# smoggy-P/gym-Drone2D-ActivePerception

Hardware: NVIDIA B200
Metric: env-steps/sec (higher is better)
Workload: dtype f64

## Files before the change

### gym_drone2d_activeperception_b200/csrc/d2d_step.cuh

```cuda
#pragma once
#include "d2d_state.cuh"
#include "d2d_math.cuh"

#if defined(D2D_COLD_NOINLINE) && D2D_COLD_NOINLINE
#define D2D_COLD __noinline__
#else
#define D2D_COLD __forceinline__
#endif

__device__ __forceinline__ uint32_t d2d_smem_u32(const void *p) { return (uint32_t)__cvta_generic_to_shared(p); }
__device__ __forceinline__ void d2d_mbar_init(uint64_t *bar, uint32_t count) {
    asm volatile("mbarrier.init.shared::cta.b64 [%0], %1;" ::"r"(d2d_smem_u32(bar)), "r"(count) : "memory");
    asm volatile("fence.mbarrier_init.release.cluster;" ::: "memory");
}
__device__ __forceinline__ void d2d_mbar_expect_tx(uint64_t *bar, uint32_t bytes) {
    asm volatile("mbarrier.arrive.expect_tx.shared::cta.b64 _, [%0], %1;" ::"r"(d2d_smem_u32(bar)), "r"(bytes) : "memory");
}
__device__ __forceinline__ void d2d_bulk_g2s(void *dst_smem, const void *src_gmem, uint32_t bytes, uint64_t *bar) {
    asm volatile("cp.async.bulk.shared::cluster.global.mbarrier::complete_tx::bytes [%0], [%1], %2, [%3];" ::"r"(
                     d2d_smem_u32(dst_smem)),
                 "l"(src_gmem), "r"(bytes), "r"(d2d_smem_u32(bar))
                 : "memory");
}
__device__ __forceinline__ void d2d_mbar_wait(uint64_t *bar, uint32_t parity) {
    uint32_t ok;
    const uint32_t addr = d2d_smem_u32(bar);
    do {
        asm volatile(
            "{ .reg .pred p; mbarrier.try_wait.parity.shared::cta.b64 p, [%1], %2; selp.u32 %0, 1, 0, p; }"
            : "=r"(ok)
            : "r"(addr), "r"(parity)
            : "memory");
    } while (!ok);
}

// ... 17 lines not shown
    int *misc;
};

__host__ __device__ inline size_t d2d_step_smem_bytes(int E, int NP, int HW) {
    size_t b = (size_t)E * D2D_BELIEF_STRIDE + (size_t)E * D2D_GT_ROW_BYTES;
    b += (size_t)E * NP * 8 * 5;
    b += ((size_t)E * NP * 2 + 15) / 16 * 16;
    b += ((size_t)E * HW * 4 + 15) / 16 * 16;
    b = (b + 15) / 16 * 16;
    b += (size_t)E * sizeof(EnvS);
    b += 16 + 16;
    return b;
}

__device__ __forceinline__ BlockCtx d2d_carve(unsigned char *base, int E, int NP, int HW) {
    BlockCtx c;
    size_t o = 0;
    c.belief = base; o += (size_t)E * D2D_BELIEF_STRIDE;
    c.gt = (uint64_t *)(base + o); o += (size_t)E * D2D_GT_ROW_BYTES;
    c.sx = (double *)(base + o); o += (size_t)E * NP * 8;
    c.sy = (double *)(base + o); o += (size_t)E * NP * 8;
    c.sr2 = (double *)(base + o); o += (size_t)E * NP * 8;
    c.mx = (double *)(base + o); o += (size_t)E * NP * 8;
    c.my = (double *)(base + o); o += (size_t)E * NP * 8;
    c.cull = (uint16_t *)(base + o); o += ((size_t)E * NP * 2 + 15) / 16 * 16;
    c.hitw = (uint32_t *)(base + o); o += ((size_t)E * HW * 4 + 15) / 16 * 16;
    o = (o + 15) / 16 * 16;
    c.S = (EnvS *)(base + o); o += (size_t)E * sizeof(EnvS);
    c.mbar = (uint64_t *)(base + o); o += 16;
    c.misc = (int *)(base + o);
    return c;
}

__device__ __forceinline__ void d2d_env_begin(const DevP &P, EnvS &s, bool was_done) {
    const bool rs = s.pending_reset != 0 || (P.auto_reset && was_done);
    s.ox_was_fresh = s.ox_fresh; s.owl_was_fresh = s.owl_fresh;
    s.pending_reset = 0; s.ox_fresh = 0; s.owl_fresh = 0;
    if (rs) {
        s.px = s.p0x; s.py = s.p0y; s.yaw = s.p0yaw; s.vx = 0; s.vy = 0; s.tgx = s.p0x; s.tgy = s.p0y;
        s.steps = 0; s.sm = SM_WAIT_FOR_GOAL; s.fail = 0; s.tcur = 0; s.bufc = 0; s.bufts = 0; s.tracked = 0;
        s.nseg = 0; s.cursor = 0;
        if (P.planner == D2D_PLANNER_JERK) { s.tgx = 0.0; s.tgy = 0.0; }
    }
    s.ix = d2d_cell(s.px, P.scale, P.inv_scale); s.iy = d2d_cell(s.py, P.scale, P.inv_scale);
    s.valid = 1; s.reset = rs; s.jerk_has = 0;
    s.ncull = 0; s.coll_agent = 0; s.arch_cnt = 0; s.arch_ts = 0; s.act_cnt = 0; s.act_ts = 0; s.newly = 0; s.done_now = 0;
}

__device__ D2D_COLD void d2d_load_env_scalars(const DevP &P, EnvS &s, int e) {
    if (e >= P.B) {
        s.valid = 0; s.reset = 0; s.done_now = 0; s.ncull = 0; s.coll_agent = 0;
        return;
    }
    const bool was_done = P.done[e] != 0;
    const uint4 *src = (const uint4 *)(P.rec + e);
    uint4 r[8];
#pragma unroll
    for (int i = 0; i < 8; i++) r[i] = src[i];
#pragma unroll
    for (int i = 0; i < 8; i++) ((uint4 *)&s)[i] = r[i];
    d2d_env_begin(P, s, was_done);
}

__device__ D2D_COLD void d2d_store_env_scalars(const DevP &P, const EnvS &s, int e) {
    uint4 *dst = (uint4 *)(P.rec + e);
#pragma unroll
    for (int i = 0; i < 8; i++) dst[i] = ((const uint4 *)&s)[i];
}

__device__ __forceinline__ void d2d_load_env_warp(const DevP &P, EnvS &s, int e, int lane) {
    unsigned long long w = 0ull;
    uint8_t was_done = 0;
    if (lane < 16) w = ((const unsigned long long *)(P.rec + e))[lane];
    if (lane == 0) was_done = P.done[e];
    if (lane < 16) ((unsigned long long *)&s)[lane] = w;
    __syncwarp();
    if (lane == 0) d2d_env_begin(P, s, was_done != 0);
// ... 152 lines not shown
#endif
    P.belief[(size_t)o.e * D2D_BELIEF_STRIDE + cell] = v;
    if (o.patch) {
        const int ci = cell / D2D_GRID, cj = cell - ci * D2D_GRID;
        const int u = ci - o.wi, w = cj - o.wj;
        if ((unsigned)u < (unsigned)D2D_LOCAL && (unsigned)w < (unsigned)D2D_LOCAL) {
            const size_t off = (size_t)o.e * D2D_LOCAL_CELLS + u * D2D_LOCAL + w;
            P.local_map[off] = v;
            if (P.lm_mirror && !o.defer_mirror) {
                P.lm_mirror[off] = v;
                atomicAdd((int *)(o.bel_s + D2D_MIRCNT_OFF), 1);
            }
        }
    }
    if (o.chg) {
        const int slot = atomicAdd(o.nchg, 1);
        if (slot < D2D_CHG_CAP) o.chg[slot] = (uint32_t)cell | ((uint32_t)v << 16);
    }
}
__device__ __forceinline__ void d2d_mark(const DevP &P, const RayOut &o, int ci, int cj, uint8_t v) {
    const int cell = ci * D2D_GRID + cj;
    if (o.bel_s[cell] != v) d2d_mark_store(P, o, cell, v);
}

__device__ __forceinline__ double d2d_ray_angle(const DevP &P, double yaw, int ray) {
    const double ray_angle = P.ray_a0 + P.ray_da * (double)ray;
    const double player_angle = D2D_TWO_PI - yaw * D2D_DEG2RAD;
    double a = player_angle + ray_angle;
    a = copysign(d2d_pymod(fabs(a), D2D_TWO_PI), a);
    if (a < 0) a += D2D_TWO_PI;
    return a;
}

template <bool SAFE = false>
__device__ __forceinline__ uint32_t d2d_cast_ray(const DevP &P, const EnvS &s, double a, double slope, const RayOut &o,
                                                 const uint64_t *gt, const double *sx, const double *sy, const double *sr2,
                                                 const uint16_t *cull, uint32_t *hitw) {
    uint32_t hm = 0u;
    const bool faced_right = (a < 90.0 * D2D_DEG2RAD) || (a > 270.0 * D2D_DEG2RAD);
    const bool faced_up = a > D2D_PI;
    const double step = P.scale - 1.0;
    double xs, ys;
    if (fabs(slope) > 1.0) {
        slope = 1.0 / slope;
        ys = faced_up ? -step : step;
        xs = ys * slope;
    } else {
        xs = faced_right ? step : -step;
        ys = xs * slope;
    }
    const double x0 = s.px, y0 = s.py;
    const int nc = s.ncull;
    uint32_t cmask = 0u;
    int mlo = 0x7fff, mhi = -1;
    {
        const double dd2 = xs * xs + ys * ys;
        const float inv_dd2 = 1.0f / (float)dd2;
        const int ncm = nc < 32 ? nc : 32;
#pragma unroll 1
        for (int q = 0; q < ncm; q++) {
            const int k = cull[q];
            const double cx = sx[k] - x0, cy = sy[k] - y0;
            const double cr = cx * ys - cy * xs;
            const double rr = sr2[k] * 1.000001 + 1e-3;
            if (cr * cr <= rr * dd2) {
                cmask |= 1u << q;
                const float t = (float)(cx * xs + cy * ys) * inv_dd2;
                const float hw = sqrtf((float)rr * inv_dd2) + 0.05f;
                mlo = min(mlo, (int)ceilf(t - hw));
                mhi = max(mhi, (int)floorf(t + hw));
            }
        }
        if (nc > 32) { mlo = 0; mhi = 0x7fff; }
    }
    const unsigned mspan = mhi >= mlo ? (unsigned)(mhi - mlo) : 0u;
    if (SAFE) {
        const bool xup = xs > 0.0, yup = ys > 0.0;
        int dcx = xup ? D2D_GRID : -D2D_GRID, dcy = yup ? 1 : -1;
        asm volatile("" : "+r"(dcx), "+r"(dcy));
        const double uxs = fabs(xs), uys = fabs(ys);
        const double ux0 = xup ? x0 : -x0, uy0 = yup ? y0 : -y0;
        double ux = ux0, uy = uy0;
        double uxb = xup ? P.scale * (double)(s.ix + 1) : -(P.scale * (double)s.ix);
        double uyb = yup ? P.scale * (double)(s.iy + 1) : -(P.scale * (double)s.iy);
        const double scale = P.scale;
        const uint32_t bel0 = d2d_smem_u32(o.bel_s);
        uint32_t caddr = bel0 + (uint32_t)(s.ix * D2D_GRID + s.iy);
        int m = 0;
        for (;;) {
            if ((unsigned)(m - mlo) <= mspan) {
                const double x = dcx > 0 ? ux : -ux, y = dcy > 0 ? uy : -uy;
                if (!(0.0 < x && 0.0 < y)) break;
                bool any = false;
                uint32_t mm = cmask;
                while (mm) {
                    const int q = __ffs(mm) - 1;
                    mm &= mm - 1u;
                    const int k = cull[q];
                    const double ex = sx[k] - x, ey = sy[k] - y;
                    if (ex * ex + ey * ey <= sr2[k]) { hm |= 1u << q; any = true; }
                }
#pragma unroll 1
                for (int q = 32; q < nc; q++) {
                    const int k = cull[q];
                    const double ex = sx[k] - x, ey = sy[k] - y;
                    if (ex * ex + ey * ey <= sr2[k]) { atomicOr(&hitw[k >> 5], 1u << (k & 31)); any = true; }
                }
                if (any) break;
            }
            uint32_t bel;
            asm volatile("ld.shared.u8 %0, [%1];" : "=r"(bel) : "r"(caddr));
            if (bel != 2u) {
                if (bel == 1u) break;
                const int cell = (int)(caddr - bel0);
                const int ci = cell / D2D_GRID, cj = cell - ci * D2D_GRID;
                if ((gt[ci] >> cj) & 1ull) {
                    bool in_map = true;
                    if (ci == 0 || cj == 0) {
                        const double x = dcx > 0 ? ux : -ux, y = dcy > 0 ? uy : -uy;
                        in_map = 0.0 < x && 0.0 < y;
                    }
                    if (in_map) d2d_mark_store(P, o, cell, 1);
                    break;
                }
                if (m >= P.m_far) {
                    const double fx = ux - ux0, fy = uy - uy0;
                    if ((fx * fx + fy * fy) >= P.depth2) break;
                }
                d2d_mark_store(P, o, cell, 2);
            } else if (m >= P.m_far) {
                const double fx = ux - ux0, fy = uy - uy0;
                if ((fx * fx + fy * fy) >= P.depth2) break;
            }
            m += 1;
            asm("{\n\t"
                ".reg .pred pe, pn;\n\t"
                "add.rn.f64 %0, %0, %3;\n\t"
                "setp.lt.s32 pn, %4, 0;\n\t"
                "setp.eq.and.f64 pe, %0, %1, pn;\n\t"
// ... 14 lines not shown
#if defined(D2D_WARP_PROF) && D2D_WARP_PROF >= 2
        atomicAdd(&P.prof[(size_t)o.e * 12 + 6], (unsigned long long)(m + 1));
        atomicMax(&P.prof[(size_t)o.e * 12 + 7], (unsigned long long)(m + 1));
#endif
        return hm;
    }
    int ci = s.ix, cj = s.iy;
    const bool xup = xs > 0.0, yup = ys > 0.0;
    const int sxi = xup ? 1 : -1, syi = yup ? 1 : -1;
    const double uxs = fabs(xs), uys = fabs(ys);
    double ux = xup ? x0 : -x0, uy = yup ? y0 : -y0;
    double uxb = xup ? P.scale * (double)(ci + 1) : -(P.scale * (double)ci);
    double uyb = yup ? P.scale * (double)(cj + 1) : -(P.scale * (double)cj);
    int m = 0;
    for (;;) {
        if ((unsigned)(ci - 1) >= (unsigned)(D2D_GRID - 2) || (unsigned)(cj - 1) >= (unsigned)(D2D_GRID - 2)) {
            const double x = xup ? ux : -ux, y = yup ? uy : -uy;
            if (!(0.0 < x && x < P.map_w && 0.0 < y && y < P.map_h)) break;
        }
        if ((unsigned)(m - mlo) <= mspan) {
            const double x = xup ? ux : -ux, y = yup ? uy : -uy;
            bool any = false;
            uint32_t mm = cmask;
            while (mm) {
                const int q = __ffs(mm) - 1;
                mm &= mm - 1u;
                const int k = cull[q];
                const double ex = sx[k] - x, ey = sy[k] - y;
                if (ex * ex + ey * ey <= sr2[k]) {
                    hm |= 1u << q;
                    any = true;
                }
            }
#pragma unroll 1
            for (int q = 32; q < nc; q++) {
                const int k = cull[q];
                const double ex = sx[k] - x, ey = sy[k] - y;
                if (ex * ex + ey * ey <= sr2[k]) {
                    atomicOr(&hitw[k >> 5], 1u << (k & 31));
                    any = true;
                }
            }
            if (any) break;
        }
        const bool wall = (gt[ci] >> cj) & 1ull;
        bool far = false;
        if (m >= P.m_far) {
            const double fx = ux - (xup ? x0 : -x0), fy = uy - (yup ? y0 : -y0);
            far = (fx * fx + fy * fy) >= P.depth2;
        }
        if (wall || far) {
            if (wall) d2d_mark(P, o, ci, cj, 1);
            break;
        }
        d2d_mark(P, o, ci, cj, 2);
        ux = ux + uxs;
        uy = uy + uys;
        m += 1;
        bool cx = ux >= uxb, cy = uy >= uyb;
        if (ux == uxb || uy == uyb) {
            if (ux == uxb && !xup) cx = false;
            if (uy == uyb && !yup) cy = false;
        }
        if (cx) { ci += sxi; uxb += P.scale; }
        if (cy) { cj += syi; uyb += P.scale; }
    }
    return hm;
}

__device__ __forceinline__ void d2d_publish_hits(uint32_t hm, const uint16_t *cull, uint32_t *hitw) {
    while (hm) {
        const int q = __ffs(hm) - 1;
        hm &= hm - 1u;
        const int k = cull[q];
        atomicOr(&hitw[k >> 5], 1u << (k & 31));
    }
}

__device__ __forceinline__ void d2d_phase_rays(const DevP &P, const BlockCtx &c, int env0, int E, int tid, int T) {
    const int R = P.n_rays, NP = P.NP;
    for (int w = tid; w < E * R; w += T) {
        const int i = w / R, ray = w - i * R;
        const EnvS &s = c.S[i];
        if (!s.valid) continue;
        RayOut o;
        o.bel_s = c.belief + (size_t)i * D2D_BELIEF_STRIDE;
        o.e = env0 + i; o.patch = 0; o.wi = 0; o.wj = 0; o.border_ok = 0; o.chg = nullptr; o.nchg = nullptr; o.defer_mirror = 0;
        const double a = d2d_ray_angle(P, s.yaw, ray);
        const uint32_t hm = d2d_cast_ray(P, s, a, d2d_tan(a), o, c.gt + (size_t)i * D2D_GRID, c.sx + i * NP, c.sy + i * NP,
                                         c.sr2 + i * NP, c.cull + i * NP, c.hitw + i * P.HW);
        d2d_publish_hits(hm, c.cull + i * NP, c.hitw + i * P.HW);
    }
}

__device__ __forceinline__ int d2d_border_intact(const uint64_t *gt, int lane) {
    const uint64_t FULL = (1ull << D2D_GRID) - 1ull, EDGE = 1ull | (1ull << (D2D_GRID - 1));
    bool ok = true;
#pragma unroll
    for (int r = lane; r < D2D_GRID; r += 32) {
        const uint64_t need = (r == 0 || r == D2D_GRID - 1) ? FULL : EDGE;
        ok = ok && ((gt[r] & need) == need);
    }
    return __all_sync(0xffffffffu, ok) ? 1 : 0;
}

template <bool ILP2>
__device__ __forceinline__ void d2d_phase_rays_warp(const DevP &P, const BlockCtx &c, const RayOut &o, int lane) {
    const EnvS &s = c.S[0];
    const int R = P.n_rays;
    uint32_t hm = 0u;
    if (ILP2) {
        for (int r0 = lane; r0 < R; r0 += 64) {
            const int r1 = r0 + 32;
            const double a0 = d2d_ray_angle(P, s.yaw, r0), a1 = d2d_ray_angle(P, s.yaw, r1);
            const double t0 = d2d_tan(a0), t1 = d2d_tan(a1);
            hm |= d2d_cast_ray(P, s, a0, t0, o, c.gt, c.sx, c.sy, c.sr2, c.cull, c.hitw);
            if (r1 < R) hm |= d2d_cast_ray(P, s, a1, t1, o, c.gt, c.sx, c.sy, c.sr2, c.cull, c.hitw);
        }
    } else {
        const bool safe = o.border_ok && (unsigned)s.ix < (unsigned)D2D_GRID && (unsigned)s.iy < (unsigned)D2D_GRID;
#pragma unroll 1
        for (int ray = lane; ray < R; ray += 32) {
            const double a = d2d_ray_angle(P, s.yaw, ray);
            const double tn = d2d_tan(a);
            if (safe) hm |= d2d_cast_ray<true>(P, s, a, tn, o, c.gt, c.sx, c.sy, c.sr2, c.cull, c.hitw);
            else hm |= d2d_cast_ray<false>(P, s, a, tn, o, c.gt, c.sx, c.sy, c.sr2, c.cull, c.hitw);
        }
    }
    hm = __reduce_or_sync(0xffffffffu, hm);
    if ((hm >> lane) & 1u) {
        const int k = c.cull[lane];
        atomicOr(&c.hitw[k >> 5], 1u << (k & 31));
    }
}

struct D2DRng {
    uint32_t *key;
    int pos, has;
    double gauss;
};
__device__ __noinline__ void d2d_mt_regen(uint32_t *mt) {
    const uint32_t UP = 0x80000000u, LO = 0x7fffffffu, MA = 0x9908b0dfu;
    int kk;
    uint32_t y;
#pragma unroll 1
    for (kk = 0; kk < 624 - 397; kk++) { y = (mt[kk] & UP) | (mt[kk + 1] & LO); mt[kk] = mt[kk + 397] ^ (y >> 1) ^ ((y & 1u) ? MA : 0u); }
#pragma unroll 1
    for (; kk < 623; kk++) { y = (mt[kk] & UP) | (mt[kk + 1] & LO); mt[kk] = mt[kk + (397 - 624)] ^ (y >> 1) ^ ((y & 1u) ? MA : 0u); }
    y = (mt[623] & UP) | (mt[0] & LO); mt[623] = mt[396] ^ (y >> 1) ^ ((y & 1u) ? MA : 0u);
}
__device__ __forceinline__ uint32_t d2d_mt_next32(D2DRng &r) {
    if (r.pos == 624) { d2d_mt_regen(r.key); r.pos = 0; }
    uint32_t y = r.key[r.pos++];
    y ^= (y >> 11); y ^= (y << 7) & 0x9d2c5680u; y ^= (y << 15) & 0xefc60000u; y ^= (y >> 18);
    return y;
}
__device__ __forceinline__ double d2d_mt_next_double(D2DRng &r) {
    const int a = (int)(d2d_mt_next32(r) >> 5), b = (int)(d2d_mt_next32(r) >> 6);
    return ((double)a * 67108864.0 + (double)b) / 9007199254740992.0;
}
__device__ __noinline__ double d2d_legacy_gauss(D2DRng &r) {
    if (r.has) { const double t = r.gauss; r.has = 0; r.gauss = 0.0; return t; }
    double f, x1, x2, r2;
    do {
        x1 = 2.0 * d2d_mt_next_double(r) - 1.0;
        x2 = 2.0 * d2d_mt_next_double(r) - 1.0;
// ... 560 lines not shown
        __syncwarp();
    }
    if (lane == 0) {
        s.tgx = -1.0; s.tgy = -1.0;
        d2d_leader_finish(P, s, c.gt, e, action, true);
        d2d_leader_flags(P, s, c.gt, e, shit);
        if (e == 0) atomicAdd(&P.stats[D2D_STAT_ENV_STEPS], (unsigned long long)P.B);
        if (!GATED && patch && P.lm_mirror) {
            const int nb = *(const int *)(c.belief + D2D_MIRCNT_OFF);
            if (nb) atomicAdd(&P.stats[D2D_STAT_MIRROR_BYTES], (unsigned long long)nb);
        }
    }
    __syncwarp();
    D2D_PROF(9);
    const int n_changed = mirror ? *nchg : 0;
    const bool rewrite = !patch || s.ix != s.obs_ix || s.iy != s.obs_iy || (mirror && n_changed > D2D_CHG_CAP);
    __syncwarp();
    if (rewrite && lane == 0) { s.obs_ix = s.ix; s.obs_iy = s.iy; }
    __syncwarp();
    d2d_store_env_warp(P, s, e, lane);
    if (rewrite) d2d_obs_env_warp(P, c.belief, s.ix, s.iy, e, lane);
    else if (mirror && n_changed > 0) {
        for (int q = lane; q < n_changed; q += 32) {
            const int cell = (int)(chg[q] & 0xFFFFu);
            const int ci = cell / D2D_GRID, cj = cell - ci * D2D_GRID;
            P.lm_mirror[(size_t)e * D2D_LOCAL_CELLS + (ci - ro.wi) * D2D_LOCAL + (cj - ro.wj)] = (uint8_t)(chg[q] >> 16);
        }
        if (lane == 0) atomicAdd(&P.stats[D2D_STAT_MIRROR_BYTES], (unsigned long long)n_changed);
    }
    if (s.done_now) d2d_count_explored_warp(P, c.belief, lane);
    D2D_PROF(3);
}

#define D2D_GATE_STAMP_SLOT(B) ((size_t)(B))

template <int WPB, int MINB, bool SYNC, bool GATED>
__global__ void __launch_bounds__(WPB * 32, MINB) d2d_rollout_warp_kernel(const DevP P, const double *__restrict__ actions,
                                                                          int K, long long action_stride, int sync_every,
                                                                          unsigned int t_first) {
    extern __shared__ __align__(128) unsigned char smem[];
    const int lane = threadIdx.x & 31, wid = threadIdx.x >> 5;
    const int e = blockIdx.x * WPB + wid;
    if (GATED) {
        if (threadIdx.x == 0) *(int *)(smem + (size_t)WPB * d2d_warp_slice_bytes(P.NP, P.HW, D2D_FUSED_WARP_EXTRA)) = 0;
        __syncthreads();
    }
    if (GATED && P.gate_src && blockIdx.x == gridDim.x - 1) {
        unsigned long long &cst = *(unsigned long long *)(smem + (size_t)WPB * d2d_warp_slice_bytes(P.NP, P.HW, D2D_FUSED_WARP_EXTRA) + 128);
        const volatile unsigned long long *hs = (const volatile unsigned long long *)P.gate_stamp_host;
        for (unsigned int t = 0;; t++) {
            if (threadIdx.x == 0) {
                const unsigned long long want = (unsigned long long)(t_first + t);
                const long long t0 = clock64();
                unsigned long long st;
                while ((((st = *hs) >> 1) & 0xffffffffull) != want) {
                    if (clock64() - t0 > 4000000000ll) { *P.gate_fault = 1u; st = (want << 1) | (1ull << 62); break; }
                }
                cst = st;
            }
            __syncthreads();
            const unsigned long long st = cst;
            const bool zero = (st >> 62) & 1ull;
#pragma unroll 1
            for (int i0 = threadIdx.x; i0 < P.B; i0 += 8 * (int)blockDim.x) {
                unsigned long long v[8];
#pragma unroll
                for (int k = 0; k < 8; k++) {
                    const int i = i0 + k * (int)blockDim.x;
                    v[k] = (i < P.B && !zero) ? __ldcv(P.gate_src + i) : 0ull;
                }
#pragma unroll
                for (int k = 0; k < 8; k++) {
                    const int i = i0 + k * (int)blockDim.x;
                    if (i < P.B) P.gate[i] = v[k];
                }
            }
            __syncthreads();
            if (threadIdx.x == 0) {
                __threadfence();
                *(volatile unsigned long long *)(P.gate + D2D_GATE_STAMP_SLOT(P.B)) = st & 0x1ffffffffull;
            }
            if (!(st & 1ull)) return;
        }
    }
    if (e >= P.B) {
        if (SYNC) for (int t = 1; t < K; t++) if (t % sync_every == 0) __syncthreads();
        return;
    }
    unsigned char *slice = smem + (size_t)wid * d2d_warp_slice_bytes(P.NP, P.HW, GATED ? D2D_FUSED_WARP_EXTRA : 0);
    const BlockCtx c = d2d_carve(slice, 1, P.NP, P.HW);
    uint32_t *chg = (uint32_t *)(slice + d2d_step_smem_bytes(1, P.NP, P.HW));
    int *nchg = (int *)(chg + D2D_CHG_CAP);
    unsigned char *blk = smem + (size_t)WPB * d2d_warp_slice_bytes(P.NP, P.HW, GATED ? D2D_FUSED_WARP_EXTRA : 0);
    int *blk_cnt = (int *)blk;
    unsigned int *blk_yaw = (unsigned int *)(blk + 16);
    unsigned int *blk_done = (unsigned int *)(blk + 16 + WPB * 4);
    const int blk_envs = min(WPB, P.B - (int)blockIdx.x * WPB);
    EnvS &s = c.S[0];
    const size_t ga = (size_t)e * P.NP + lane;
    double2 pf_pos = double2{0.0, 0.0}, pf_pref = double2{0.0, 0.0};
    double pf_r = 0.0;
    uint8_t pf_act = 0;
    if (lane < P.N) {
        pf_pos = P.apos[ga]; pf_pref = P.apref[ga]; pf_r = P.arad[ga];
        if (P.trackers) pf_act = P.trk_active[ga];
    }
    double action = GATED ? 0.0 : actions[e];
    if (lane == 0) {
        if (GATED) *nchg = 0;
        d2d_mbar_init(c.mbar, 1);
        d2d_mbar_expect_tx(c.mbar, D2D_GT_ROW_BYTES + D2D_BELIEF_STRIDE);
        d2d_bulk_g2s(c.gt, P.gt_rows + (size_t)e * D2D_GRID, D2D_GT_ROW_BYTES, c.mbar);
        d2d_bulk_g2s(c.belief, P.belief + (size_t)e * D2D_BELIEF_STRIDE, D2D_BELIEF_STRIDE, c.mbar);
        c.misc[0] = 0;
    }
    d2d_load_env_warp(P, s, e, lane);
    if (lane == 0) c.misc[1] = s.reset;
#pragma unroll 1
    for (int w = lane; w < P.HW; w += 32) c.hitw[w] = 0u;
    __syncwarp();
    int border_ok = 0;
    const bool mirror = GATED && P.lm_mirror != nullptr;
#pragma unroll 1
    for (int t = 0;;) {
        D2D_PROF(0);
        d2d_reset_prefetch(P, s, e, lane, pf_pos, pf_pref);
        d2d_reset_arrays(P, c, e, 1, lane, 32, t == 0 ? c.mbar : nullptr);
        d2d_phase_agents<true, true>(P, c, e, 1, lane, 32, pf_pos, pf_pref, pf_r, &pf_pos, &pf_pref);
        if (t == 0 && pf_act && !s.reset) d2d_prefetch_tracker(P, ga);
        if (lane == 0) d2d_leader_begin(P, s);
        __syncwarp();
        const bool refill = s.reset && s.obs_ix == s.ix && s.obs_iy == s.iy && (GATED || P.lm_mirror == nullptr);
        const bool patch = (!s.reset || refill) && s.obs_ix == s.ix && s.obs_iy == s.iy;
        if (refill) d2d_obs_clear_warp(P, e, lane, false);
        RayOut ro;
        ro.bel_s = c.belief; ro.e = e; ro.patch = patch ? 1 : 0;
        ro.wi = s.ix - 16; ro.wj = s.iy - 16;
        ro.chg = (mirror && patch && !refill) ? chg : nullptr; ro.nchg = nchg; ro.defer_mirror = GATED ? 1 : 0;
        if (t == 0) {
            d2d_mbar_wait(c.mbar, 0);
            border_ok = d2d_border_intact(c.gt, lane);
        }
        ro.border_ok = border_ok;
        D2D_PROF(1);
        d2d_phase_rays_warp<false>(P, c, ro, lane);
        __syncwarp();
        D2D_PROF(2);
        if (P.var_cam != 0.0) {
            if (lane == 0) d2d_measure_env(P, c, e);
            __syncwarp();
        }
        d2d_phase_trackers<true>(P, c, e, 1, lane, 32, pf_act);
        const int shit = __any_sync(0xffffffffu, lane < 5 ? d2d_static_probe(P, c.gt, s.px, s.py, lane) : 0);
        __syncwarp();
        int more = (t + 1 < K) ? 1 : 0;
        bool rewrite = false;
        int n_changed = 0;
        if (GATED) {
            if (lane == 0) {
                s.tgx = -1.0; s.tgy = -1.0;
                d2d_leader_finish(P, s, c.gt, e, 0.0, true, false);
                d2d_leader_flags(P, s, c.gt, e, shit, false);
            }
            __syncwarp();
            n_changed = (mirror && !refill) ? *nchg : 0;
            rewrite = !patch || s.ix != s.obs_ix || s.iy != s.obs_iy || (mirror && n_changed > D2D_CHG_CAP);
            __syncwarp();
            if (rewrite && lane == 0) { s.obs_ix = s.ix; s.obs_iy = s.iy; }
            __syncwarp();
            if (rewrite) d2d_obs_env_warp(P, c.belief, s.ix, s.iy, e, lane, false);
            if (s.done_now) d2d_count_explored_warp(P, c.belief, lane);
            D2D_PROF(8);
            if (lane == 0) {
                volatile unsigned long long *slot = P.gate + e;
                volatile unsigned long long *stamp = P.gate + D2D_GATE_STAMP_SLOT(P.B);
                const unsigned long long want = (unsigned long long)(t_first + (unsigned int)t);
                const long long t0 = clock64();
                unsigned long long bits, st = 0ull;
                bool fault = false;
                while ((bits = *slot) == D2D_ACTION_SENTINEL) {
                    if (clock64() - t0 > 4000000000ll) { fault = true; break; }
                }
                if (!fault) {
                    while (((st = *stamp) >> 1) != want) {
                        if (clock64() - t0 > 4000000000ll) { fault = true; break; }
                    }
                }
                if (fault) { *P.gate_fault = 1u; bits = 0ull; st = 0ull; }
                action = __longlong_as_double((long long)bits);
                *slot = D2D_ACTION_SENTINEL;
                more = (int)(st & 1ull);
                s.yaw = d2d_pymod(s.yaw + (action * P.max_yaw_speed) * P.dt, 360.0);
                P.yaw_obs[e] = (float)s.yaw;
            }
            more = __shfl_sync(0xffffffffu, more, 0);
            D2D_PROF(9);
            if (mirror) {
                if (rewrite || refill) {
                    __syncwarp();
                    d2d_obs_mirror_copy_warp(P, e, lane);
                } else if (n_changed > 0) {
                    for (int q = lane; q < n_changed; q += 32) {
                        const int cell = (int)(chg[q] & 0xFFFFu);
                        const int ci = cell / D2D_GRID, cj = cell - ci * D2D_GRID;
                        P.lm_mirror[(size_t)e * D2D_LOCAL_CELLS + (ci - ro.wi) * D2D_LOCAL + (cj - ro.wj)] = (uint8_t)(chg[q] >> 16);
                    }
                    if (lane == 0) atomicAdd(&P.stats[D2D_STAT_MIRROR_BYTES], (unsigned long long)n_changed);
                }
            }
            __syncwarp();
        } else {
            if (lane == 0) {
                s.tgx = -1.0; s.tgy = -1.0;
                d2d_leader_finish(P, s, c.gt, e, action, true);
                d2d_leader_flags(P, s, c.gt, e, shit);
                if (patch && P.lm_mirror) {
                    int *cnt = (int *)(c.belief + D2D_MIRCNT_OFF);
                    const int nb = *cnt;
                    if (nb) { atomicAdd(&P.stats[D2D_STAT_MIRROR_BYTES], (unsigned long long)nb); *cnt = 0; }
                }
            }
            __syncwarp();
            rewrite = !patch || s.ix != s.obs_ix || s.iy != s.obs_iy;
            __syncwarp();
            if (rewrite && lane == 0) { s.obs_ix = s.ix; s.obs_iy = s.iy; }
            __syncwarp();
            if (rewrite) d2d_obs_env_warp(P, c.belief, s.ix, s.iy, e, lane);
            if (s.done_now) d2d_count_explored_warp(P, c.belief, lane);
        }
        D2D_PROF(4);
        if (GATED) {
            int last = 0;
            if (lane == 0) {
                atomicExch(&blk_yaw[wid], __float_as_uint((float)s.yaw)); atomicExch(&blk_done[wid], (unsigned int)s.done_now);
                __threadfence_block();
                last = atomicAdd(blk_cnt, 1) == blk_envs - 1 ? 1 : 0;
            }
            last = __shfl_sync(0xffffffffu, last, 0);
            if (last) {
                __threadfence_block();
                const int e0 = (int)blockIdx.x * WPB;
                if (lane < blk_envs) {
                    if (P.yaw_mirror) P.yaw_mirror[e0 + lane] = __uint_as_float(atomicOr(&blk_yaw[lane], 0u));
                    if (P.done_mirror) P.done_mirror[e0 + lane] = (uint8_t)atomicOr(&blk_done[lane], 0u);
                }
                __syncwarp();
                if (lane == 0) {
                    *blk_cnt = 0;
                    __threadfence();
                    const unsigned long long n = atomicAdd(P.gate_count, (unsigned long long)blk_envs) + (unsigned long long)blk_envs;
                    if (n == (unsigned long long)P.B * (unsigned long long)(t + 1)) {
                        atomicAdd(&P.stats[D2D_STAT_ENV_STEPS], (unsigned long long)P.B);
                        asm volatile("fence.acq_rel.sys;" ::: "memory");
                        *(volatile unsigned int *)P.gate_done = t_first + (unsigned int)t;
                    }
                }
            }
        }
        D2D_PROF(3);
        t += 1;
        if (!more) break;
        if (SYNC && t % sync_every == 0) __syncthreads();
        if (!GATED) action = actions[(size_t)t * (size_t)action_stride + e];
        if (P.trackers && lane < P.N) pf_act = P.trk_active[ga];
#pragma unroll 1
        for (int w = lane; w < P.HW; w += 32) c.hitw[w] = 0u;
        __syncwarp();
        if (lane == 0) {
            const bool was_done = s.done_now != 0;
            d2d_env_begin(P, s, was_done);
            c.misc[1] = s.reset;
            if (GATED) *nchg = 0;
        }
        __syncwarp();
    }
    d2d_store_env_warp(P, s, e, lane);
    if (!GATED && e == 0 && lane == 0) atomicAdd(&P.stats[D2D_STAT_ENV_STEPS], (unsigned long long)P.B * (unsigned long long)K);
}
```

### gym_drone2d_activeperception_b200/csrc/drone2d.cu

```cuda
#include <cstddef>
#include <cstdio>
#include <cstdlib>
#include <cstring>
#include <cmath>
#include <string>
#include <vector>
#include <initializer_list>

#include "d2d_state.cuh"
#include "d2d_math.cuh"
#include "d2d_step.cuh"
#include "d2d_plan.cuh"
#include "d2d_rvo.cuh"
#include "d2d_clone.cuh"
#include "d2d_worldgen.cuh"
#include "d2d_episode.cuh"
#include "d2d_render.cuh"
#include "d2d_difficulty.cuh"

struct EnvRows {
    int64_t row_bytes, row_stride;
    int planes;
    int64_t plane_stride;
};
// ... 926 lines not shown
    } else if (h->cfg.planner == D2D_PLANNER_JERK) {
        if (!h->jerk_set) { h->err = "planner = Jerk_Primitive: d2d_set_jerk_tables must provide the heading tables"; return D2D_ERR_STATE; }
        rc = launch_jerk_warp<4>(h, actions_dev, st);
    } else {
        rc = step_primitive(h, actions_dev, st);
    }
    if (rc != D2D_OK) return rc;
    CUDA_TRY(h, cudaGetLastError());
    return D2D_OK;
}

static int launch_prim_warp_entry(d2d_handle *h, const double *actions, cudaStream_t st, double *ox_next);

extern "C" int d2d_step_plan_oxford(d2d_handle *h, const double *actions_dev, double *next_actions_dev, void *stream) {
    if (!h || !actions_dev || !next_actions_dev) return D2D_ERR_INVALID;
    D2D_NO_PIPE(h);
    if (!h->world_set) { h->err = "d2d_step_plan_oxford before d2d_set_world"; return D2D_ERR_STATE; }
    if (!(h->cfg.oxford & D2D_POLICY_OXFORD)) { h->err = "d2d_step_plan_oxford: handle was created without the Oxford state (cfg.oxford & 1)"; return D2D_ERR_STATE; }
    if (h->cfg.var_cam != 0.0 && !h->rng_set) { h->err = "var_cam != 0: d2d_set_rng must provide the np.random stream state"; return D2D_ERR_STATE; }
    if (h->cfg.planner != D2D_PLANNER_PRIMITIVE || h->cfg.envs_per_block > 0 || h->P.motion_rvo) {
        int rc = step_impl(h, actions_dev, stream);
        if (rc == D2D_OK) rc = d2d_plan_oxford(h, next_actions_dev, stream);
        return rc != D2D_OK ? rc : log_step(h, (cudaStream_t)stream);
    }
    CUDA_TRY(h, cudaSetDevice(h->cfg.device));
    const int rc = launch_prim_warp_entry(h, actions_dev, (cudaStream_t)stream, next_actions_dev);
    if (rc != D2D_OK) return rc;
    CUDA_TRY(h, cudaGetLastError());
    return log_step(h, (cudaStream_t)stream);
}

#define D2D_RESIDENT_WPB 28

template <int WPB, int MINB, bool SYNC, bool GATED>
static int launch_rollout(d2d_handle *h, const double *actions, int K, long long stride, cudaStream_t st, unsigned int t_first = 0,
                          int extra_blocks = 0) {
    const size_t smem = (size_t)WPB * d2d_warp_slice_bytes(h->NP, h->HW, GATED ? D2D_FUSED_WARP_EXTRA : 0) + (GATED ? 256 : 0);
    if (smem > 227 * 1024) { h->err = "rollout kernel: shared memory per block exceeds 227 KB"; return D2D_ERR_INVALID; }
    const int rc = ensure_smem_attr(h, (const void *)d2d_rollout_warp_kernel<WPB, MINB, SYNC, GATED>, "rollout warp");
    if (rc != D2D_OK) return rc;
    static const int sync_every = getenv("D2D_ROLLOUT_SYNC") ? atoi(getenv("D2D_ROLLOUT_SYNC")) : 1;
    d2d_rollout_warp_kernel<WPB, MINB, SYNC, GATED><<<(h->B + WPB - 1) / WPB + extra_blocks, WPB * 32, smem, st>>>(
        h->P, actions, K, stride, sync_every > 0 ? sync_every : 1, t_first);
    return D2D_OK;
}

static int resident_capacity(d2d_handle *h) {
    if (h->resident_capacity >= 0) return h->resident_capacity;
    constexpr int WPB = D2D_RESIDENT_WPB;
    const size_t smem = (size_t)WPB * d2d_warp_slice_bytes(h->NP, h->HW, D2D_FUSED_WARP_EXTRA) + 256;
    int cap = 0, nb = 0, sms = 0;
    if (smem <= 227 * 1024 && ensure_smem_attr(h, (const void *)d2d_rollout_warp_kernel<WPB, 1, false, true>, "rollout warp") == D2D_OK &&
        cudaOccupancyMaxActiveBlocksPerMultiprocessor(&nb, d2d_rollout_warp_kernel<WPB, 1, false, true>, WPB * 32, smem) == cudaSuccess &&
        cudaDeviceGetAttribute(&sms, cudaDevAttrMultiProcessorCount, h->cfg.device) == cudaSuccess)
        { cap = nb * sms * WPB; h->resident_blocks = nb * sms; }
    else
        cudaGetLastError();
    if (getenv("D2D_PIPE_DEBUG")) fprintf(stderr, "[d2d pipelined] resident kernel: %d blocks/SM x %d SMs, smem %zu B -> capacity %d envs (%s)\n", nb, sms, smem, cap, cudaGetErrorString(cudaPeekAtLastError()));
    h->resident_capacity = cap;
    return cap;
}

extern "C" int d2d_rollout(d2d_handle *h, const double *actions_dev, int32_t num_steps, int64_t action_stride, void *stream) {
    if (!h || !actions_dev || num_steps < 1) return D2D_ERR_INVALID;
    D2D_NO_PIPE(h);
    if (!h->world_set) { h->err = "d2d_rollout before d2d_set_world"; return D2D_ERR_STATE; }
    if (h->cfg.var_cam != 0.0 && !h->rng_set) { h->err = "var_cam != 0: d2d_set_rng must provide the np.random stream state"; return D2D_ERR_STATE; }
    if (h->cfg.planner != D2D_PLANNER_NOMOVE || h->P.motion_rvo || h->cfg.envs_per_block > 0) {
        h->err = "d2d_rollout: NoMove planner, CVM motion profile and the default warp kernels only (use d2d_step)";
        return D2D_ERR_INVALID;
    }
    if (action_stride != 0 && action_stride < h->B) { h->err = "d2d_rollout: action_stride must be 0 or >= num_envs"; return D2D_ERR_INVALID; }
    CUDA_TRY(h, cudaSetDevice(h->cfg.device));
    cudaStream_t st = (cudaStream_t)stream;
    static const int variant = getenv("D2D_ROLLOUT_VARIANT") ? atoi(getenv("D2D_ROLLOUT_VARIANT")) : 0;
    int rc;
    if ((variant == 0 && h->B > 2 * 28 * 148) || h->ep_mem) {
        for (int t = 0; t < num_steps; t++) {
            rc = launch_fused_warp<4, 7, false>(h, actions_dev + (size_t)t * (size_t)action_stride, st);
            if (rc == D2D_OK) rc = log_step(h, st);
            if (rc != D2D_OK) return rc;
        }
        CUDA_TRY(h, cudaGetLastError());
        return D2D_OK;
    }
    switch (variant) {
        case 1: rc = launch_rollout<4, 7, false, false>(h, actions_dev, num_steps, action_stride, st); break;
        case 2: rc = launch_rollout<4, 7, true, false>(h, actions_dev, num_steps, action_stride, st); break;
        case 3: rc = launch_rollout<7, 4, true, false>(h, actions_dev, num_steps, action_stride, st); break;
        case 4: rc = launch_rollout<14, 2, true, false>(h, actions_dev, num_steps, action_stride, st); break;
        default: rc = launch_rollout<28, 1, true, false>(h, actions_dev, num_steps, action_stride, st); break;
    }
    if (rc != D2D_OK) return rc;
    h->launches++;
    CUDA_TRY(h, cudaGetLastError());
    return D2D_OK;
}

extern "C" int d2d_step_host(d2d_handle *h, const double *actions_host, uint8_t *local_map_host, float *yaw_host,
                             uint8_t *done_host, void *stream) {
    if (!h) return D2D_ERR_INVALID;
    CUDA_TRY(h, cudaSetDevice(h->cfg.device));
    cudaStream_t st = (cudaStream_t)stream;
    const double *act = actions_host ? nullptr : h->stage_actions;
    if (actions_host) {
        cudaPointerAttributes at;
        if (cudaPointerGetAttributes(&at, actions_host) == cudaSuccess && at.type == cudaMemoryTypeHost && at.devicePointer)
            act = (const double *)at.devicePointer;
        else
            cudaGetLastError();
    }
    if (!act) {
        CUDA_TRY(h, cudaMemcpyAsync(h->stage_actions, actions_host, (size_t)h->B * 8, cudaMemcpyHostToDevice, st));
        act = h->stage_actions;
    }
    int rc = d2d_step(h, act, stream);
    if (rc != D2D_OK) return rc;
    const bool fresh = !h->mir_stale;
    if (local_map_host && !(fresh && local_map_host == h->mir_lm))
        CUDA_TRY(h, cudaMemcpyAsync(local_map_host, h->P.local_map, (size_t)h->B * D2D_LOCAL_CELLS, cudaMemcpyDeviceToHost, st));
    if (yaw_host && !(fresh && yaw_host == h->mir_yaw))
        CUDA_TRY(h, cudaMemcpyAsync(yaw_host, h->P.yaw_obs, (size_t)h->B * 4, cudaMemcpyDeviceToHost, st));
    if (done_host && !(fresh && done_host == h->mir_done))
        CUDA_TRY(h, cudaMemcpyAsync(done_host, h->P.done, (size_t)h->B, cudaMemcpyDeviceToHost, st));
// ... 654 lines not shown
```

Baseline: 233.1 million.

## Add specialized small-crowd rollout kernel path for at most 32 agents

Adds a SMALL template variant of the warp rollout kernel used when agent count fits in one warp. Each lane owns one agent, so culling uses a ballot, hit masks come back as a warp register instead of shared-memory atomics, and the per-step hitw clear and overflow loops are dropped. The shared-memory slice shrinks, static probing runs only on reset, and a dedicated no-move leader finish is used. The catch is a separate code path whose episode and stats semantics must stay identical to the general path.

```diff
diff --git a/gym_drone2d_activeperception_b200/csrc/d2d_step.cuh b/gym_drone2d_activeperception_b200/csrc/d2d_step.cuh
--- a/gym_drone2d_activeperception_b200/csrc/d2d_step.cuh
+++ b/gym_drone2d_activeperception_b200/csrc/d2d_step.cuh
@@ -1,6 +1,7 @@
 #pragma once
 #include "d2d_state.cuh"
 #include "d2d_math.cuh"
+#include "d2d_agent_math.cuh"
 
 #if defined(D2D_COLD_NOINLINE) && D2D_COLD_NOINLINE
 #define D2D_COLD __noinline__
@@ -84,6 +85,7 @@
     return c;
 }
 
+template <bool CELL = true>
 __device__ __forceinline__ void d2d_env_begin(const DevP &P, EnvS &s, bool was_done) {
     const bool rs = s.pending_reset != 0 || (P.auto_reset && was_done);
     s.ox_was_fresh = s.ox_fresh; s.owl_was_fresh = s.owl_fresh;
@@ -94,7 +96,7 @@
         s.nseg = 0; s.cursor = 0;
         if (P.planner == D2D_PLANNER_JERK) { s.tgx = 0.0; s.tgy = 0.0; }
     }
-    s.ix = d2d_cell(s.px, P.scale, P.inv_scale); s.iy = d2d_cell(s.py, P.scale, P.inv_scale);
+    if (CELL) { s.ix = d2d_cell(s.px, P.scale, P.inv_scale); s.iy = d2d_cell(s.py, P.scale, P.inv_scale); }
     s.valid = 1; s.reset = rs; s.jerk_has = 0;
     s.ncull = 0; s.coll_agent = 0; s.arch_cnt = 0; s.arch_ts = 0; s.act_cnt = 0; s.act_ts = 0; s.newly = 0; s.done_now = 0;
 }
@@ -313,7 +315,7 @@
     return a;
 }
 
-template <bool SAFE = false>
+template <bool SAFE = false, bool SMALL = false>
 __device__ __forceinline__ uint32_t d2d_cast_ray(const DevP &P, const EnvS &s, double a, double slope, const RayOut &o,
                                                  const uint64_t *gt, const double *sx, const double *sy, const double *sr2,
                                                  const uint16_t *cull, uint32_t *hitw) {
@@ -337,7 +339,7 @@
     {
         const double dd2 = xs * xs + ys * ys;
         const float inv_dd2 = 1.0f / (float)dd2;
-        const int ncm = nc < 32 ? nc : 32;
+        const int ncm = (SMALL || nc < 32) ? nc : 32;
 #pragma unroll 1
         for (int q = 0; q < ncm; q++) {
             const int k = cull[q];
@@ -352,7 +354,7 @@
                 mhi = max(mhi, (int)floorf(t + hw));
             }
         }
-        if (nc > 32) { mlo = 0; mhi = 0x7fff; }
+        if (!SMALL && nc > 32) { mlo = 0; mhi = 0x7fff; }
     }
     const unsigned mspan = mhi >= mlo ? (unsigned)(mhi - mlo) : 0u;
     if (SAFE) {
@@ -381,11 +383,13 @@
                     const double ex = sx[k] - x, ey = sy[k] - y;
                     if (ex * ex + ey * ey <= sr2[k]) { hm |= 1u << q; any = true; }
                 }
-#pragma unroll 1
-                for (int q = 32; q < nc; q++) {
-                    const int k = cull[q];
-                    const double ex = sx[k] - x, ey = sy[k] - y;
-                    if (ex * ex + ey * ey <= sr2[k]) { atomicOr(&hitw[k >> 5], 1u << (k & 31)); any = true; }
+                if (!SMALL) {
+#pragma unroll 1
+                    for (int q = 32; q < nc; q++) {
+                        const int k = cull[q];
+                        const double ex = sx[k] - x, ey = sy[k] - y;
+                        if (ex * ex + ey * ey <= sr2[k]) { atomicOr(&hitw[k >> 5], 1u << (k & 31)); any = true; }
+                    }
                 }
                 if (any) break;
             }
@@ -466,13 +470,15 @@
                     any = true;
                 }
             }
-#pragma unroll 1
-            for (int q = 32; q < nc; q++) {
-                const int k = cull[q];
-                const double ex = sx[k] - x, ey = sy[k] - y;
-                if (ex * ex + ey * ey <= sr2[k]) {
-                    atomicOr(&hitw[k >> 5], 1u << (k & 31));
-                    any = true;
+            if (!SMALL) {
+#pragma unroll 1
+                for (int q = 32; q < nc; q++) {
+                    const int k = cull[q];
+                    const double ex = sx[k] - x, ey = sy[k] - y;
+                    if (ex * ex + ey * ey <= sr2[k]) {
+                        atomicOr(&hitw[k >> 5], 1u << (k & 31));
+                        any = true;
+                    }
                 }
             }
             if (any) break;
@@ -538,8 +544,9 @@
     return __all_sync(0xffffffffu, ok) ? 1 : 0;
 }
 
-template <bool ILP2>
-__device__ __forceinline__ void d2d_phase_rays_warp(const DevP &P, const BlockCtx &c, const RayOut &o, int lane) {
+template <bool ILP2, bool SMALL = false>
+__device__ __forceinline__ uint32_t d2d_phase_rays_warp(const DevP &P, const BlockCtx &c, const RayOut &o, int lane) {
+    static_assert(!(ILP2 && SMALL), "the small-crowd form casts one ray per lane per pass");
     const EnvS &s = c.S[0];
     const int R = P.n_rays;
     uint32_t hm = 0u;
@@ -557,15 +564,17 @@
         for (int ray = lane; ray < R; ray += 32) {
             const double a = d2d_ray_angle(P, s.yaw, ray);
             const double tn = d2d_tan(a);
-            if (safe) hm |= d2d_cast_ray<true>(P, s, a, tn, o, c.gt, c.sx, c.sy, c.sr2, c.cull, c.hitw);
-            else hm |= d2d_cast_ray<false>(P, s, a, tn, o, c.gt, c.sx, c.sy, c.sr2, c.cull, c.hitw);
+            if (safe) hm |= d2d_cast_ray<true, SMALL>(P, s, a, tn, o, c.gt, c.sx, c.sy, c.sr2, c.cull, c.hitw);
+            else hm |= d2d_cast_ray<false, SMALL>(P, s, a, tn, o, c.gt, c.sx, c.sy, c.sr2, c.cull, c.hitw);
         }
     }
     hm = __reduce_or_sync(0xffffffffu, hm);
+    if (SMALL) return __reduce_or_sync(0xffffffffu, ((hm >> lane) & 1u) ? 1u << c.cull[lane] : 0u);
     if ((hm >> lane) & 1u) {
         const int k = c.cull[lane];
         atomicOr(&c.hitw[k >> 5], 1u << (k & 31));
     }
+    return 0u;
 }
 
 struct D2DRng {
@@ -1192,12 +1201,91 @@
     D2D_PROF(3);
 }
 
+
+__device__ __forceinline__ bool d2d_agents_lane(const DevP &P, const BlockCtx &c, EnvS &s, size_t g, int lane, double2 &pos,
+                                                double2 &pref, double r) {
+    bool in = false, hit = false;
+    if (lane < P.N) {
+        d2d_cvm_agent_step(pos.x, pos.y, pref.x, pref.y, r, P.dt, P.scale, P.map_w, P.map_h);
+        P.apos[g] = pos;
+        P.apref[g] = pref;
+        c.sx[lane] = pos.x; c.sy[lane] = pos.y; c.sr2[lane] = r * r;
+        const double ddx = pos.x - s.px, ddy = pos.y - s.py;
+        const double reach = r + P.cull_reach;
+        in = ddx * ddx + ddy * ddy <= reach * reach;
+        hit = d2d_norm2_lt(ddx, ddy, r + P.drone_r);
+    }
+    const uint32_t b = __ballot_sync(0xffffffffu, in);
+    if (in) c.cull[__popc(b & ((1u << lane) - 1u))] = (uint16_t)lane;
+    if (lane == 0) s.ncull = __popc(b);
+    return __any_sync(0xffffffffu, hit);
+}
+
+__device__ __forceinline__ void d2d_trackers_lane(const DevP &P, const BlockCtx &c, EnvS &s, size_t g, int lane, uint32_t hmask,
+                                                  uint8_t pf_act) {
+    if (lane >= P.N) return;
+    const bool hit = (hmask >> lane) & 1u;
+    P.hit[g] = hit ? 1 : 0;
+    if (P.trackers) {
+        const bool was_active = !s.reset && pf_act != 0;
+        if (hit && !was_active) atomicAdd(&s.newly, 1);
+        if (was_active || hit || s.reset) {
+            const bool noisy = P.var_cam != 0.0;
+            d2d_tracker_update(P, s, g, hit, noisy ? c.mx[lane] : c.sx[lane], noisy ? c.my[lane] : c.sy[lane], was_active);
+        }
+    }
+}
+
+__device__ __forceinline__ void d2d_leader_nomove(const DevP &P, EnvS &s, const uint64_t *gt, int e, double action, bool coll,
+                                                  int &inv) {
+    const int shit = inv & 1;
+    bool goal = (inv & 2) != 0;
+    s.tgx = -1.0; s.tgy = -1.0;
+    if (s.nseg * P.n_way - s.cursor > 0) {
+        d2d_leader_finish(P, s, gt, e, 0.0, true, false);
+        s.ix = d2d_cell(s.px, P.scale, P.inv_scale); s.iy = d2d_cell(s.py, P.scale, P.inv_scale);
+        goal = d2d_norm2_le(s.px - s.tgx, s.py - s.tgy, 10.0);
+        int sh = 0;
+        for (int q = 0; q < 5; q++) sh |= d2d_static_probe(P, gt, s.px, s.py, q);
+        inv = sh | (goal ? 2 : 0);
+    } else {
+        s.sm = SM_EXECUTING; s.fail = 0;
+    }
+    s.yaw = d2d_pymod(s.yaw + (action * P.max_yaw_speed) * P.dt, 360.0);
+    const int col = shit ? 1 : (coll ? 2 : 0);
+    int frz = 0;
+    if (col == 0) {
+        if (goal) s.sm = SM_GOAL_REACHED;
+        frz = ((double)s.steps >= P.max_steps) ? 1 : 0;
+    }
+    const int done = (col != 0 || frz || (s.sm == SM_GOAL_REACHED && s.tcur >= P.n_targets)) ? 1 : 0;
+    s.bufc += s.arch_cnt; s.bufts += s.arch_ts; s.tracked += s.newly;
+    if (done) { s.bufc += s.act_cnt; s.bufts += s.act_ts; }
+    s.done_now = done;
+    P.collision[e] = (uint8_t)col; P.dead_lock[e] = 0; P.freezing[e] = (uint8_t)frz; P.done[e] = (uint8_t)done;
+    P.yaw_obs[e] = (float)s.yaw;
+    if (P.yaw_mirror) P.yaw_mirror[e] = (float)s.yaw;
+    if (P.done_mirror) P.done_mirror[e] = (uint8_t)done;
+    if (done) {
+        atomicAdd(&P.stats[D2D_STAT_EPISODES], 1ull);
+        if (s.sm == SM_GOAL_REACHED) atomicAdd(&P.stats[D2D_STAT_SUCCESS], 1ull);
+        if (col == 1) atomicAdd(&P.stats[D2D_STAT_STATIC_COLLISION], 1ull);
+        if (col == 2) atomicAdd(&P.stats[D2D_STAT_DYNAMIC_COLLISION], 1ull);
+        if (frz) atomicAdd(&P.stats[D2D_STAT_FREEZING], 1ull);
+        atomicAdd(&P.stats[D2D_STAT_FLIGHT_STEPS], (unsigned long long)s.steps);
+        atomicAdd(&P.stats[D2D_STAT_AGENTS_TRACKED], (unsigned long long)s.bufc);
+        atomicAdd(&P.stats[D2D_STAT_TRACKED_STEPS], (unsigned long long)s.bufts);
+    }
+}
+
 #define D2D_GATE_STAMP_SLOT(B) ((size_t)(B))
-
-template <int WPB, int MINB, bool SYNC, bool GATED>
+#define D2D_SMALL_N 32
+
+template <int WPB, int MINB, bool SYNC, bool GATED, bool SMALL = false>
 __global__ void __launch_bounds__(WPB * 32, MINB) d2d_rollout_warp_kernel(const DevP P, const double *__restrict__ actions,
                                                                           int K, long long action_stride, int sync_every,
                                                                           unsigned int t_first) {
+    static_assert(!(SMALL && GATED), "the small-crowd form serves d2d_rollout only");
     extern __shared__ __align__(128) unsigned char smem[];
     const int lane = threadIdx.x & 31, wid = threadIdx.x >> 5;
     const int e = blockIdx.x * WPB + wid;
@@ -1247,11 +1335,13 @@
         if (SYNC) for (int t = 1; t < K; t++) if (t % sync_every == 0) __syncthreads();
         return;
     }
-    unsigned char *slice = smem + (size_t)wid * d2d_warp_slice_bytes(P.NP, P.HW, GATED ? D2D_FUSED_WARP_EXTRA : 0);
-    const BlockCtx c = d2d_carve(slice, 1, P.NP, P.HW);
-    uint32_t *chg = (uint32_t *)(slice + d2d_step_smem_bytes(1, P.NP, P.HW));
+    unsigned char *slice = smem + (size_t)wid * d2d_warp_slice_bytes(SMALL ? D2D_SMALL_N : P.NP, SMALL ? 1 : P.HW,
+                                                                     GATED ? D2D_FUSED_WARP_EXTRA : 0);
+    const BlockCtx c = d2d_carve(slice, 1, SMALL ? D2D_SMALL_N : P.NP, SMALL ? 1 : P.HW);
+    uint32_t *chg = (uint32_t *)(slice + d2d_step_smem_bytes(1, SMALL ? D2D_SMALL_N : P.NP, SMALL ? 1 : P.HW));
     int *nchg = (int *)(chg + D2D_CHG_CAP);
-    unsigned char *blk = smem + (size_t)WPB * d2d_warp_slice_bytes(P.NP, P.HW, GATED ? D2D_FUSED_WARP_EXTRA : 0);
+    unsigned char *blk = smem + (size_t)WPB * d2d_warp_slice_bytes(SMALL ? D2D_SMALL_N : P.NP, SMALL ? 1 : P.HW,
+                                                                   GATED ? D2D_FUSED_WARP_EXTRA : 0);
     int *blk_cnt = (int *)blk;
     unsigned int *blk_yaw = (unsigned int *)(blk + 16);
     unsigned int *blk_done = (unsigned int *)(blk + 16 + WPB * 4);
@@ -1276,20 +1366,40 @@
     }
     d2d_load_env_warp(P, s, e, lane);
     if (lane == 0) c.misc[1] = s.reset;
-#pragma unroll 1
-    for (int w = lane; w < P.HW; w += 32) c.hitw[w] = 0u;
+    if (!SMALL) {
+#pragma unroll 1
+        for (int w = lane; w < P.HW; w += 32) c.hitw[w] = 0u;
+    }
     __syncwarp();
     int border_ok = 0;
     const bool mirror = GATED && P.lm_mirror != nullptr;
+    int inv = 0;
 #pragma unroll 1
     for (int t = 0;;) {
         D2D_PROF(0);
         d2d_reset_prefetch(P, s, e, lane, pf_pos, pf_pref);
         d2d_reset_arrays(P, c, e, 1, lane, 32, t == 0 ? c.mbar : nullptr);
-        d2d_phase_agents<true, true>(P, c, e, 1, lane, 32, pf_pos, pf_pref, pf_r, &pf_pos, &pf_pref);
+        bool coll = false;
+        if (SMALL) coll = d2d_agents_lane(P, c, s, ga, lane, pf_pos, pf_pref, pf_r);
+        else d2d_phase_agents<true, true>(P, c, e, 1, lane, 32, pf_pos, pf_pref, pf_r, &pf_pos, &pf_pref);
         if (t == 0 && pf_act && !s.reset) d2d_prefetch_tracker(P, ga);
         if (lane == 0) d2d_leader_begin(P, s);
         __syncwarp();
+        if (SMALL) {
+            if (t == 0) {
+                d2d_mbar_wait(c.mbar, 0);
+                border_ok = d2d_border_intact(c.gt, lane);
+            }
+            if (t == 0 || s.reset) {
+                const double px = s.px, py = s.py;
+                const int sh = __any_sync(0xffffffffu, lane < 5 ? d2d_static_probe(P, c.gt, px, py, lane) : 0);
+                if (lane == 0) {
+                    inv = sh | (d2d_norm2_le(px - -1.0, py - -1.0, 10.0) ? 2 : 0);
+                    s.ix = d2d_cell(px, P.scale, P.inv_scale); s.iy = d2d_cell(py, P.scale, P.inv_scale);
+                }
+                __syncwarp();
+            }
+        }
         const bool refill = s.reset && s.obs_ix == s.ix && s.obs_iy == s.iy && (GATED || P.lm_mirror == nullptr);
         const bool patch = (!s.reset || refill) && s.obs_ix == s.ix && s.obs_iy == s.iy;
         if (refill) d2d_obs_clear_warp(P, e, lane, false);
@@ -1297,21 +1407,25 @@
         ro.bel_s = c.belief; ro.e = e; ro.patch = patch ? 1 : 0;
         ro.wi = s.ix - 16; ro.wj = s.iy - 16;
         ro.chg = (mirror && patch && !refill) ? chg : nullptr; ro.nchg = nchg; ro.defer_mirror = GATED ? 1 : 0;
-        if (t == 0) {
+        if (!SMALL && t == 0) {
             d2d_mbar_wait(c.mbar, 0);
             border_ok = d2d_border_intact(c.gt, lane);
         }
         ro.border_ok = border_ok;
         D2D_PROF(1);
-        d2d_phase_rays_warp<false>(P, c, ro, lane);
+        const uint32_t hmask = d2d_phase_rays_warp<false, SMALL>(P, c, ro, lane);
         __syncwarp();
         D2D_PROF(2);
         if (P.var_cam != 0.0) {
-            if (lane == 0) d2d_measure_env(P, c, e);
+            if (lane == 0) {
+                if (SMALL) c.hitw[0] = hmask;
+                d2d_measure_env(P, c, e);
+            }
             __syncwarp();
         }
-        d2d_phase_trackers<true>(P, c, e, 1, lane, 32, pf_act);
-        const int shit = __any_sync(0xffffffffu, lane < 5 ? d2d_static_probe(P, c.gt, s.px, s.py, lane) : 0);
+        if (SMALL) d2d_trackers_lane(P, c, s, ga, lane, hmask, pf_act);
+        else d2d_phase_trackers<true>(P, c, e, 1, lane, 32, pf_act);
+        const int shit = SMALL ? 0 : __any_sync(0xffffffffu, lane < 5 ? d2d_static_probe(P, c.gt, s.px, s.py, lane) : 0);
         __syncwarp();
         int more = (t + 1 < K) ? 1 : 0;
         bool rewrite = false;
@@ -1371,9 +1485,12 @@
             __syncwarp();
         } else {
             if (lane == 0) {
-                s.tgx = -1.0; s.tgy = -1.0;
-                d2d_leader_finish(P, s, c.gt, e, action, true);
-                d2d_leader_flags(P, s, c.gt, e, shit);
+                if (SMALL) d2d_leader_nomove(P, s, c.gt, e, action, coll, inv);
+                else {
+                    s.tgx = -1.0; s.tgy = -1.0;
+                    d2d_leader_finish(P, s, c.gt, e, action, true);
+                    d2d_leader_flags(P, s, c.gt, e, shit);
+                }
                 if (patch && P.lm_mirror) {
                     int *cnt = (int *)(c.belief + D2D_MIRCNT_OFF);
                     const int nb = *cnt;
@@ -1423,12 +1540,14 @@
         if (SYNC && t % sync_every == 0) __syncthreads();
         if (!GATED) action = actions[(size_t)t * (size_t)action_stride + e];
         if (P.trackers && lane < P.N) pf_act = P.trk_active[ga];
-#pragma unroll 1
-        for (int w = lane; w < P.HW; w += 32) c.hitw[w] = 0u;
+        if (!SMALL) {
+#pragma unroll 1
+            for (int w = lane; w < P.HW; w += 32) c.hitw[w] = 0u;
+        }
         __syncwarp();
         if (lane == 0) {
             const bool was_done = s.done_now != 0;
-            d2d_env_begin(P, s, was_done);
+            d2d_env_begin<!SMALL>(P, s, was_done);
             c.misc[1] = s.reset;
             if (GATED) *nchg = 0;
         }
diff --git a/gym_drone2d_activeperception_b200/csrc/drone2d.cu b/gym_drone2d_activeperception_b200/csrc/drone2d.cu
--- a/gym_drone2d_activeperception_b200/csrc/drone2d.cu
+++ b/gym_drone2d_activeperception_b200/csrc/drone2d.cu
@@ -982,15 +982,16 @@
 
 #define D2D_RESIDENT_WPB 28
 
-template <int WPB, int MINB, bool SYNC, bool GATED>
+template <int WPB, int MINB, bool SYNC, bool GATED, bool SMALL = false>
 static int launch_rollout(d2d_handle *h, const double *actions, int K, long long stride, cudaStream_t st, unsigned int t_first = 0,
                           int extra_blocks = 0) {
-    const size_t smem = (size_t)WPB * d2d_warp_slice_bytes(h->NP, h->HW, GATED ? D2D_FUSED_WARP_EXTRA : 0) + (GATED ? 256 : 0);
+    const size_t smem = (size_t)WPB * d2d_warp_slice_bytes(SMALL ? D2D_SMALL_N : h->NP, SMALL ? 1 : h->HW,
+                                                           GATED ? D2D_FUSED_WARP_EXTRA : 0) + (GATED ? 256 : 0);
     if (smem > 227 * 1024) { h->err = "rollout kernel: shared memory per block exceeds 227 KB"; return D2D_ERR_INVALID; }
-    const int rc = ensure_smem_attr(h, (const void *)d2d_rollout_warp_kernel<WPB, MINB, SYNC, GATED>, "rollout warp");
+    const int rc = ensure_smem_attr(h, (const void *)d2d_rollout_warp_kernel<WPB, MINB, SYNC, GATED, SMALL>, "rollout warp");
     if (rc != D2D_OK) return rc;
     static const int sync_every = getenv("D2D_ROLLOUT_SYNC") ? atoi(getenv("D2D_ROLLOUT_SYNC")) : 1;
-    d2d_rollout_warp_kernel<WPB, MINB, SYNC, GATED><<<(h->B + WPB - 1) / WPB + extra_blocks, WPB * 32, smem, st>>>(
+    d2d_rollout_warp_kernel<WPB, MINB, SYNC, GATED, SMALL><<<(h->B + WPB - 1) / WPB + extra_blocks, WPB * 32, smem, st>>>(
         h->P, actions, K, stride, sync_every > 0 ? sync_every : 1, t_first);
     return D2D_OK;
 }
@@ -1039,7 +1040,9 @@
         case 2: rc = launch_rollout<4, 7, true, false>(h, actions_dev, num_steps, action_stride, st); break;
         case 3: rc = launch_rollout<7, 4, true, false>(h, actions_dev, num_steps, action_stride, st); break;
         case 4: rc = launch_rollout<14, 2, true, false>(h, actions_dev, num_steps, action_stride, st); break;
-        default: rc = launch_rollout<28, 1, true, false>(h, actions_dev, num_steps, action_stride, st); break;
+        default: rc = h->N <= D2D_SMALL_N ? launch_rollout<28, 1, true, false, true>(h, actions_dev, num_steps, action_stride, st)
+                                          : launch_rollout<28, 1, true, false>(h, actions_dev, num_steps, action_stride, st);
+                 break;
     }
     if (rc != D2D_OK) return rc;
     h->launches++;
```

New measurement: 243.7 million (median of 6 runs). 4.5% higher.
